# rat-and-catcher/in_cwave

Measured on AMD Instinct MI355X. Metric: Msamples/s through Hilbert+mod+render, higher is better.
Workload: dtype f64

## Files before the change

in_cwave_amd/csrc/icw_iir_dev.h:

```cpp
#ifndef ICW_IIR_DEV_H_
#define ICW_IIR_DEV_H_

#pragma clang fp contract(off)

template <int J>
__device__ __forceinline__ double icw_chain_x(double v, bool qodd)
{
    return (((J & 1) != 0) != qodd) ? 0.0 : v;
}

__device__ __forceinline__ double icw_minabs(double m, double s)
{
    double r;
    asm("v_min_f64 %0, %1, |%2|" : "=v"(r) : "v"(m), "v"(s));
    return r;
}

__device__ __forceinline__ double icw_minabs_v(double m, double s)
{
    double r;
    asm volatile("v_min_f64 %0, %1, |%2|" : "=v"(r) : "v"(m), "v"(s));
    return r;
}

template <int N, int J>
__device__ __forceinline__ void icw_store_hist(const double (&R)[N], double *hist, int g, int n_chains)
{
#pragma unroll
    for (int i = 0; i < N; ++i) hist[(size_t)g * ICW_HIST_PITCH + i] = R[(J - 1 - i + 2 * N) % N];
}

template <int N>
__device__ __forceinline__ void icw_rotate1(double (&R)[N])
{
    const double r0 = R[0];
#pragma unroll
    for (int k = 0; k < N - 1; ++k) R[k] = R[k + 1];
    R[N - 1] = r0;
}

template <int N>
__device__ __forceinline__ void icw_normalise_ring(double (&R)[N], int rem)
{
#pragma unroll
    for (int k = 1; k < N; ++k)
        if (k <= rem) icw_rotate1<N>(R);
}

#define ICW_DRAIN_VMEM() __builtin_amdgcn_s_waitcnt(0x0F70)

template <int N>
__device__ __forceinline__ void icw_load_x(double (&xv)[N], const double *xp)
{
#pragma unroll
    for (int j = 0; j < N; ++j) xv[j] = xp[j];
}

template <int N>
__device__ __forceinline__ void icw_store_block(const double (&R)[N], double *wo)
{
#pragma unroll
    for (int j = 0; j < N; ++j) wo[j] = R[j];
}


__device__ __forceinline__ double icw_vmul(double a, double b)
{
    double r;
    asm volatile("v_mul_f64 %0, %1, %2" : "=v"(r) : "v"(a), "v"(b));
    return r;
}

#include "icw_row_asm.inc"

struct IcwRowC {
    double c0, c1;
    double pl, pl2;
    double one;
};

template <int N>
constexpr bool icw_row_c0p() { return N > 17; }
template <int N>
constexpr int icw_row_c0_lane() { return N - 17; }


template <int N, int J, int Z, bool SPEC>
__device__ __forceinline__ void icw_row_step(double (&W)[N], double (&P)[N], double (&P2)[N], double xin,
                                             double xin2, const IcwRowC &c, double &mn, bool qodd = false)
{
    if constexpr (Z == 2) xin = icw_chain_x<J>(xin, qodd);
    constexpr bool ZS = Z != 2 && (J & 1) == Z;
    constexpr bool C0P = icw_row_c0p<N>() && Z != 2 && !ZS;
    double S;
    if constexpr (C0P) {
        S = icw_row_chain<N, 0, J>(xin, 0.0, xin2, c.one, P, P2);
    } else {
        double Y;
        if constexpr (ZS) {
            S = W[(J - 1 + N) % N] * c.c0;
            Y = W[(J - 2 + 2 * N) % N] * c.c1;
        } else {
            S = xin;
            Y = W[(J - 1 + N) % N] * c.c0;
        }
        const double T = S + Y;
        double NC = Y - (T - S);
        S = icw_row_chain<N, ZS ? 2 : 1, J>(T, NC, 0.0, c.one, P, P2);
    }
    if constexpr (!SPEC) S = fabs(S) < 1.0 ? 0.0 : S;
    W[J] = S;
    if constexpr (N > 17) P2[J] = icw_vmul(c.pl2, S);
    P[J] = icw_vmul(c.pl, S);
    if constexpr (SPEC) mn = icw_minabs_v(mn, S);
    else if constexpr (icw_row_c0p<N>()) asm volatile("s_nop 1");
}

template <int N, int J, int Z, int ZN, bool SPEC>
__device__ __forceinline__ void icw_row_block(double (&W)[N], double (&P)[N], double (&P2)[N], double (&xv)[N],
                                              double (&xv2)[N], const double *xnext, const double *xnext2,
                                              const IcwRowC &c, double &mn, bool qodd = false)
{
    if constexpr (J < N) {
        icw_row_step<N, J, Z, SPEC>(W, P, P2, xv[J], xv2[J], c, mn, qodd);
        if constexpr (!(ZN != 2 && (J & 1) == ZN)) {
            xv[J] = xnext[J];
            if constexpr (icw_row_c0p<N>() && ZN != 2) xv2[J] = xnext2[J];
        }
        icw_row_block<N, J + 1, Z, ZN, SPEC>(W, P, P2, xv, xv2, xnext, xnext2, c, mn, qodd);
    }
}

template <int N, int J>
__device__ __forceinline__ void icw_row_block_lim(double (&W)[N], double (&P)[N], double (&P2)[N],
                                                  const double (&xv)[N], const IcwRowC &c, int lim, bool qodd)
{
    if constexpr (J < N) {
        if (J < lim) {
            double mn;
            icw_row_step<N, J, 2, false>(W, P, P2, xv[J], 0.0, c, mn, qodd);
            icw_row_block_lim<N, J + 1>(W, P, P2, xv, c, lim, qodd);
        }
    }
}

template <int N>
__device__ __forceinline__ void icw_row_store(const double (&W)[N], double *wo, bool writer)
{
    if (writer) {
#pragma unroll
        for (int j = 0; j < N; ++j) wo[j] = W[j];
    }
}

template <int N>
__device__ __forceinline__ void icw_row_products(const double (&W)[N], double (&P)[N], double (&P2)[N],
                                                 const IcwRowC &c)
{
    if constexpr (N > 17) {
#pragma unroll
        for (int k = 0; k < N; ++k) P2[k] = icw_vmul(c.pl2, W[k]);
    }
#pragma unroll
    for (int k = 0; k < N; ++k) P[k] = icw_vmul(c.pl, W[k]);
    asm volatile("s_nop 1");
}

template <int N>
__device__ __forceinline__ void icw_row_restart(double (&W)[N], double (&P)[N], double (&P2)[N], double (&xv)[N],
                                                double (&xv2)[N], const double *xp, const double *xp2,
                                                const double *wrow, int t, const IcwRowC &c)
{
    __builtin_amdgcn_fence(__ATOMIC_SEQ_CST, "workgroup");
#pragma unroll
    for (int j = 0; j < N; ++j) W[j] = wrow[t + j];
    icw_row_products<N>(W, P, P2, c);
    icw_load_x<N>(xv, xp + t);
    if constexpr (icw_row_c0p<N>()) icw_load_x<N>(xv2, xp2 + t);
}

template <bool PUB>
__device__ __forceinline__ void icw_row_publish(int *prog, int gl, int f, int done)
{
    if constexpr (PUB) {
        asm volatile("" ::: "memory");
        if ((gl & 63) == 0) *(volatile __attribute__((address_space(3))) int *)(prog + f) = done;
    }
}

template <int N, bool PUB = false>
__device__ __forceinline__ void icw_iir_row_body(const IcwK1Args &a, int gl, double *lw = nullptr, int lpitch = 0,
                                                 int *prog = nullptr)
{
    const int wv = gl >> 6, r = (gl >> 4) & 3, lr = gl & 15;
    const int f = wv & 1;
    const int slot = (wv >> 1) * 4 + r;
    const bool dedup = a.dedup != 0;
    const int s = dedup ? slot : (slot >> 1), ch = dedup ? 0 : (slot & 1);
    if (s >= a.n_streams) return;
    const int g = s * 4 + ch * 2 + f;
    const bool writer = lr == 0;

    IcwRowC c;
    c.c0 = a.pc[0];
    c.c1 = a.pc[1];
    c.pl = (lr + 1 < N) ? a.pc[lr + 1] : 0.0;
    c.pl2 = (lr + 17 < N) ? a.pc[lr + 17] : (icw_row_c0p<N>() && lr == icw_row_c0_lane<N>()) ? a.pc[0] : 0.0;
    c.one = 1.0;

    double W[N], P[N], P2[N];
#pragma unroll
    for (int i = 0; i < N; ++i) W[N - 1 - i] = a.hist[(size_t)g * ICW_HIST_PITCH + i];
    icw_row_products<N>(W, P, P2, c);

    if (writer && ch == 0) a.info_dup[s * 2 + f] = a.lr_equal[s * 2 + f];
    const double *xp = a.xd + (size_t)(s * 2 + ch) * a.x_pitch;
    const unsigned phi = (a.hq_phase[s * 2 + ch] + (unsigned)a.t0 + (unsigned)f) & 1u;
    int zoff = 0;
    asm volatile("" : "+s"(zoff));
    const double *xp2 = xp + zoff;
    double *wrow = PUB ? lw + (size_t)(ch * 2 + f) * lpitch : a.w + (size_t)g * a.w_pitch;
    icw_row_store<N>(W, wrow, writer);

    const int T = a.T;
    int t = 0;
    if (T >= N) {
        double xv[N], xv2[N];
        icw_load_x<N>(xv, xp);
        if constexpr (icw_row_c0p<N>()) icw_load_x<N>(xv2, xp2);
        const unsigned phi0 = __builtin_amdgcn_readfirstlane(phi);
        const bool zfast = __all(phi == phi0) && T >= 3 * N;
        double mn = __builtin_inf();
        bool fail = false;
        ICW_DRAIN_VMEM();
        if (zfast) {
            if constexpr (N & 1) {
                if ((phi0 + (unsigned)t) & 1u) {
                    icw_row_block<N, 0, 0, 1, false>(W, P, P2, xv, xv2, xp + t + N, xp2 + t + N, c, mn);
                    icw_row_store<N>(W, wrow + N + t, writer);
                    t += N;
                }
                for (; t + 2 * N <= T; t += 2 * N) {
                    icw_row_block<N, 0, 1, 0, true>(W, P, P2, xv, xv2, xp + t + N, xp2 + t + N, c, mn);
                    icw_row_store<N>(W, wrow + N + t, writer);
                    icw_row_block<N, 0, 0, 1, true>(W, P, P2, xv, xv2, xp + t + 2 * N, xp2 + t + 2 * N, c, mn);
                    icw_row_store<N>(W, wrow + 2 * N + t, writer);
                    if (__any(mn < 1.0)) { fail = true; break; }
                    icw_row_publish<PUB>(prog, gl, f, t + 2 * N);
                }
            } else if (phi0) {
                for (; t + N <= T; t += N) {
                    icw_row_block<N, 0, 0, 0, true>(W, P, P2, xv, xv2, xp + t + N, xp2 + t + N, c, mn);
                    icw_row_store<N>(W, wrow + N + t, writer);
                    if (__any(mn < 1.0)) { fail = true; break; }
                    icw_row_publish<PUB>(prog, gl, f, t + N);
                }
            } else {
                for (; t + N <= T; t += N) {
                    icw_row_block<N, 0, 1, 1, true>(W, P, P2, xv, xv2, xp + t + N, xp2 + t + N, c, mn);
                    icw_row_store<N>(W, wrow + N + t, writer);
                    if (__any(mn < 1.0)) { fail = true; break; }
                    icw_row_publish<PUB>(prog, gl, f, t + N);
                }
            }
            if (fail) icw_row_restart<N>(W, P, P2, xv, xv2, xp, xp2, wrow, t, c);
            else icw_load_x<N>(xv, xp + t);
        }
        if (fail) {
            ICW_DRAIN_VMEM();
            if constexpr (N & 1) {
                if (((phi0 + (unsigned)t) & 1u) && t + N <= T) {
                    icw_row_block<N, 0, 0, 1, false>(W, P, P2, xv, xv2, xp + t + N, xp2 + t + N, c, mn);
                    icw_row_store<N>(W, wrow + N + t, writer);
                    t += N;
                }
                for (; t + 2 * N <= T; t += 2 * N) {
                    icw_row_block<N, 0, 1, 0, false>(W, P, P2, xv, xv2, xp + t + N, xp2 + t + N, c, mn);
                    icw_row_store<N>(W, wrow + N + t, writer);
                    icw_row_block<N, 0, 0, 1, false>(W, P, P2, xv, xv2, xp + t + 2 * N, xp2 + t + 2 * N, c, mn);
                    icw_row_store<N>(W, wrow + 2 * N + t, writer);
                    icw_row_publish<PUB>(prog, gl, f, t + 2 * N);
                }
            } else if (phi0) {
                for (; t + N <= T; t += N) {
                    icw_row_block<N, 0, 0, 0, false>(W, P, P2, xv, xv2, xp + t + N, xp2 + t + N, c, mn);
                    icw_row_store<N>(W, wrow + N + t, writer);
                    icw_row_publish<PUB>(prog, gl, f, t + N);
                }
            } else {
                for (; t + N <= T; t += N) {
                    icw_row_block<N, 0, 1, 1, false>(W, P, P2, xv, xv2, xp + t + N, xp2 + t + N, c, mn);
                    icw_row_store<N>(W, wrow + N + t, writer);
                    icw_row_publish<PUB>(prog, gl, f, t + N);
                }
            }
            icw_load_x<N>(xv, xp + t);
        }
        for (; t + N <= T; t += N) {
            icw_row_block<N, 0, 2, 2, false>(W, P, P2, xv, xv2, xp + t + N, xp2 + t + N, c, mn,
                                             ((phi + (unsigned)t) & 1u) != 0u);
            icw_row_store<N>(W, wrow + N + t, writer);
            icw_row_publish<PUB>(prog, gl, f, t + N);
        }
    }
    const int rem = T - t;
    if (rem > 0) {
        double xv[N];
#pragma unroll
        for (int j = 0; j < N; ++j) xv[j] = (j < rem) ? xp[t + j] : 0.0;
        icw_row_block_lim<N, 0>(W, P, P2, xv, c, rem, ((phi + (unsigned)t) & 1u) != 0u);
        if (writer) {
            double *wo = wrow + N + t;
#pragma unroll
            for (int j = 0; j < N; ++j)
                if (j < rem) wo[j] = W[j];
        }
        icw_normalise_ring<N>(W, rem);
    }
    icw_row_publish<PUB>(prog, gl, f, T);
    if (writer) {
        icw_store_hist<N, 0>(W, a.hist, g, a.n_chains);
        if (dedup) icw_store_hist<N, 0>(W, a.hist, g + 2, a.n_chains);
    }
    if (dedup) {
        if (writer) a.lr_equal[s * 2 + f] = 1u;
        return;
    }
    bool eq = true;
#pragma unroll
    for (int i = 0; i < N; ++i) {
        const double o = __shfl_xor(W[i], 16);
        eq = eq && (__double_as_longlong(o) == __double_as_longlong(W[i]));
    }
    if (writer && ch == 0) a.lr_equal[s * 2 + f] = eq ? 1u : 0u;
}

#endif
```

Baseline: 3251.

## Replace per-step min-abs speculation check with lagged reload check from stored row

In the non-publishing path, the speculative zero-skip loop no longer folds a min-abs into every recurrence step. Instead it reloads a few samples of already-stored output per iteration and checks them one or two iterations later, rolling back by two iterations on failure. This takes the extra v_min_f64 and its dependency off the serial IIR critical path. In exchange it adds memory loads, a deferred check that relies on stored values being visible to the same lane, and more rollback work when a failure occurs.

```diff
diff --git a/in_cwave_amd/csrc/icw_iir_dev.h b/in_cwave_amd/csrc/icw_iir_dev.h
--- a/in_cwave_amd/csrc/icw_iir_dev.h
+++ b/in_cwave_amd/csrc/icw_iir_dev.h
@@ -85,7 +85,9 @@
 constexpr int icw_row_c0_lane() { return N - 17; }
 
 
-template <int N, int J, int Z, bool SPEC>
+enum { ICW_SPEC_OFF = 0, ICW_SPEC_MIN = 1, ICW_SPEC_LAG = 2 };
+
+template <int N, int J, int Z, int SPEC>
 __device__ __forceinline__ void icw_row_step(double (&W)[N], double (&P)[N], double (&P2)[N], double xin,
                                              double xin2, const IcwRowC &c, double &mn, bool qodd = false)
 {
@@ -112,11 +114,13 @@
     W[J] = S;
     if constexpr (N > 17) P2[J] = icw_vmul(c.pl2, S);
     P[J] = icw_vmul(c.pl, S);
-    if constexpr (SPEC) mn = icw_minabs_v(mn, S);
-    else if constexpr (icw_row_c0p<N>()) asm volatile("s_nop 1");
-}
-
-template <int N, int J, int Z, int ZN, bool SPEC>
+    if constexpr (SPEC == ICW_SPEC_MIN) mn = icw_minabs_v(mn, S);
+    else if constexpr (SPEC == ICW_SPEC_LAG) {
+        if constexpr (icw_row_c0p<N>() && ZS) asm volatile("s_nop 0");
+    } else if constexpr (icw_row_c0p<N>()) asm volatile("s_nop 1");
+}
+
+template <int N, int J, int Z, int ZN, int SPEC>
 __device__ __forceinline__ void icw_row_block(double (&W)[N], double (&P)[N], double (&P2)[N], double (&xv)[N],
                                               double (&xv2)[N], const double *xnext, const double *xnext2,
                                               const IcwRowC &c, double &mn, bool qodd = false)
@@ -138,7 +142,7 @@
     if constexpr (J < N) {
         if (J < lim) {
             double mn;
-            icw_row_step<N, J, 2, false>(W, P, P2, xv[J], 0.0, c, mn, qodd);
+            icw_row_step<N, J, 2, ICW_SPEC_OFF>(W, P, P2, xv[J], 0.0, c, mn, qodd);
             icw_row_block_lim<N, J + 1>(W, P, P2, xv, c, lim, qodd);
         }
     }
@@ -164,6 +168,42 @@
 #pragma unroll
     for (int k = 0; k < N; ++k) P[k] = icw_vmul(c.pl, W[k]);
     asm volatile("s_nop 1");
+}
+
+template <int M>
+__device__ __forceinline__ void icw_row_chk_load(double (&q)[(M + 15) / 16], const double *p)
+{
+    constexpr int L = (M + 15) / 16;
+#pragma unroll
+    for (int i = 0; i < L; ++i)
+        q[i] = __hip_atomic_load(p + (i < L - 1 ? 16 * i : M - 16), __ATOMIC_RELAXED, __HIP_MEMORY_SCOPE_AGENT);
+}
+
+template <int L>
+__device__ __forceinline__ double icw_row_chk_fold(double mn, const double (&q)[L])
+{
+#pragma unroll
+    for (int i = 0; i < L; ++i) mn = icw_minabs_v(mn, q[i]);
+    return mn;
+}
+
+__device__ __forceinline__ double icw_minabs2_v(double a, double b)
+{
+    double r;
+    asm volatile("v_min_f64 %0, |%1|, |%2|" : "=v"(r) : "v"(a), "v"(b));
+    return r;
+}
+
+template <int M>
+__device__ __forceinline__ bool icw_row_chk_fail(double (&q)[(M + 15) / 16], const double *wq, int t, int ts)
+{
+    constexpr int L = (M + 15) / 16;
+    double m = icw_minabs2_v(q[0], q[1]);
+    if constexpr (L > 2) m = icw_minabs_v(m, q[2]);
+    static_assert(L == 2 || L == 3, "16 < samples per iteration <= 48");
+    const bool bad = t >= ts + 2 * M && __any(m < 1.0);
+    icw_row_chk_load<M>(q, wq + (t > ts ? t : ts + M));
+    return bad;
 }
 
 template <int N>
@@ -234,33 +274,69 @@
         bool fail = false;
         ICW_DRAIN_VMEM();
         if (zfast) {
+            constexpr int SP = PUB ? ICW_SPEC_MIN : ICW_SPEC_LAG;
+            constexpr int M = (N & 1) ? 2 * N : N;
+            double q[(M + 15) / 16];
+#pragma unroll
+            for (int i = 0; i < (M + 15) / 16; ++i) q[i] = __builtin_inf();
+            const double *wq = wrow + N - M + lr;
             if constexpr (N & 1) {
                 if ((phi0 + (unsigned)t) & 1u) {
-                    icw_row_block<N, 0, 0, 1, false>(W, P, P2, xv, xv2, xp + t + N, xp2 + t + N, c, mn);
+                    icw_row_block<N, 0, 0, 1, ICW_SPEC_OFF>(W, P, P2, xv, xv2, xp + t + N, xp2 + t + N, c, mn);
                     icw_row_store<N>(W, wrow + N + t, writer);
                     t += N;
                 }
+            }
+            const int ts = t;
+            if constexpr (N & 1) {
                 for (; t + 2 * N <= T; t += 2 * N) {
-                    icw_row_block<N, 0, 1, 0, true>(W, P, P2, xv, xv2, xp + t + N, xp2 + t + N, c, mn);
-                    icw_row_store<N>(W, wrow + N + t, writer);
-                    icw_row_block<N, 0, 0, 1, true>(W, P, P2, xv, xv2, xp + t + 2 * N, xp2 + t + 2 * N, c, mn);
+                    icw_row_block<N, 0, 1, 0, SP>(W, P, P2, xv, xv2, xp + t + N, xp2 + t + N, c, mn);
+                    icw_row_store<N>(W, wrow + N + t, writer);
+                    icw_row_block<N, 0, 0, 1, SP>(W, P, P2, xv, xv2, xp + t + 2 * N, xp2 + t + 2 * N, c, mn);
                     icw_row_store<N>(W, wrow + 2 * N + t, writer);
-                    if (__any(mn < 1.0)) { fail = true; break; }
-                    icw_row_publish<PUB>(prog, gl, f, t + 2 * N);
+                    if constexpr (PUB) {
+                        if (__any(mn < 1.0)) { fail = true; break; }
+                        icw_row_publish<PUB>(prog, gl, f, t + 2 * N);
+                    } else {
+                        if (icw_row_chk_fail<M>(q, wq, t, ts)) { fail = true; t -= 2 * M; break; }
+                    }
                 }
             } else if (phi0) {
                 for (; t + N <= T; t += N) {
-                    icw_row_block<N, 0, 0, 0, true>(W, P, P2, xv, xv2, xp + t + N, xp2 + t + N, c, mn);
-                    icw_row_store<N>(W, wrow + N + t, writer);
-                    if (__any(mn < 1.0)) { fail = true; break; }
-                    icw_row_publish<PUB>(prog, gl, f, t + N);
+                    icw_row_block<N, 0, 0, 0, SP>(W, P, P2, xv, xv2, xp + t + N, xp2 + t + N, c, mn);
+                    icw_row_store<N>(W, wrow + N + t, writer);
+                    if constexpr (PUB) {
+                        if (__any(mn < 1.0)) { fail = true; break; }
+                        icw_row_publish<PUB>(prog, gl, f, t + N);
+                    } else {
+                        if (icw_row_chk_fail<M>(q, wq, t, ts)) { fail = true; t -= 2 * M; break; }
+                    }
                 }
             } else {
                 for (; t + N <= T; t += N) {
-                    icw_row_block<N, 0, 1, 1, true>(W, P, P2, xv, xv2, xp + t + N, xp2 + t + N, c, mn);
-                    icw_row_store<N>(W, wrow + N + t, writer);
-                    if (__any(mn < 1.0)) { fail = true; break; }
-                    icw_row_publish<PUB>(prog, gl, f, t + N);
+                    icw_row_block<N, 0, 1, 1, SP>(W, P, P2, xv, xv2, xp + t + N, xp2 + t + N, c, mn);
+                    icw_row_store<N>(W, wrow + N + t, writer);
+                    if constexpr (PUB) {
+                        if (__any(mn < 1.0)) { fail = true; break; }
+                        icw_row_publish<PUB>(prog, gl, f, t + N);
+                    } else {
+                        if (icw_row_chk_fail<M>(q, wq, t, ts)) { fail = true; t -= 2 * M; break; }
+                    }
+                }
+            }
+            if constexpr (!PUB) {
+                if (!fail) {
+                    ICW_DRAIN_VMEM();
+                    mn = __builtin_inf();
+                    if (t >= ts + 2 * M) mn = icw_row_chk_fold(mn, q);
+                    if (t > ts) {
+                        icw_row_chk_load<M>(q, wq + t);
+                        mn = icw_row_chk_fold(mn, q);
+                    }
+                    if (__any(mn < 1.0)) {
+                        fail = true;
+                        t = (t - 2 * M > ts) ? t - 2 * M : ts;
+                    }
                 }
             }
             if (fail) icw_row_restart<N>(W, P, P2, xv, xv2, xp, xp2, wrow, t, c);
@@ -270,26 +346,26 @@
             ICW_DRAIN_VMEM();
             if constexpr (N & 1) {
                 if (((phi0 + (unsigned)t) & 1u) && t + N <= T) {
-                    icw_row_block<N, 0, 0, 1, false>(W, P, P2, xv, xv2, xp + t + N, xp2 + t + N, c, mn);
+                    icw_row_block<N, 0, 0, 1, ICW_SPEC_OFF>(W, P, P2, xv, xv2, xp + t + N, xp2 + t + N, c, mn);
                     icw_row_store<N>(W, wrow + N + t, writer);
                     t += N;
                 }
                 for (; t + 2 * N <= T; t += 2 * N) {
-                    icw_row_block<N, 0, 1, 0, false>(W, P, P2, xv, xv2, xp + t + N, xp2 + t + N, c, mn);
-                    icw_row_store<N>(W, wrow + N + t, writer);
-                    icw_row_block<N, 0, 0, 1, false>(W, P, P2, xv, xv2, xp + t + 2 * N, xp2 + t + 2 * N, c, mn);
+                    icw_row_block<N, 0, 1, 0, ICW_SPEC_OFF>(W, P, P2, xv, xv2, xp + t + N, xp2 + t + N, c, mn);
+                    icw_row_store<N>(W, wrow + N + t, writer);
+                    icw_row_block<N, 0, 0, 1, ICW_SPEC_OFF>(W, P, P2, xv, xv2, xp + t + 2 * N, xp2 + t + 2 * N, c, mn);
                     icw_row_store<N>(W, wrow + 2 * N + t, writer);
                     icw_row_publish<PUB>(prog, gl, f, t + 2 * N);
                 }
             } else if (phi0) {
                 for (; t + N <= T; t += N) {
-                    icw_row_block<N, 0, 0, 0, false>(W, P, P2, xv, xv2, xp + t + N, xp2 + t + N, c, mn);
+                    icw_row_block<N, 0, 0, 0, ICW_SPEC_OFF>(W, P, P2, xv, xv2, xp + t + N, xp2 + t + N, c, mn);
                     icw_row_store<N>(W, wrow + N + t, writer);
                     icw_row_publish<PUB>(prog, gl, f, t + N);
                 }
             } else {
                 for (; t + N <= T; t += N) {
-                    icw_row_block<N, 0, 1, 1, false>(W, P, P2, xv, xv2, xp + t + N, xp2 + t + N, c, mn);
+                    icw_row_block<N, 0, 1, 1, ICW_SPEC_OFF>(W, P, P2, xv, xv2, xp + t + N, xp2 + t + N, c, mn);
                     icw_row_store<N>(W, wrow + N + t, writer);
                     icw_row_publish<PUB>(prog, gl, f, t + N);
                 }
@@ -297,7 +373,7 @@
             icw_load_x<N>(xv, xp + t);
         }
         for (; t + N <= T; t += N) {
-            icw_row_block<N, 0, 2, 2, false>(W, P, P2, xv, xv2, xp + t + N, xp2 + t + N, c, mn,
+            icw_row_block<N, 0, 2, 2, ICW_SPEC_OFF>(W, P, P2, xv, xv2, xp + t + N, xp2 + t + N, c, mn,
                                              ((phi + (unsigned)t) & 1u) != 0u);
             icw_row_store<N>(W, wrow + N + t, writer);
             icw_row_publish<PUB>(prog, gl, f, t + N);
```

Measured after the change: 3270 (median of 6 runs). About the same (+0.6%).
